# DiltheyLab/MetaMaps

Hardware: AMD Instinct MI355X
Metric: Gbp long reads mapped+classified per sec (whole node), miniSeq+H DB (higher is better)
Workload: dtype u32

## Files before the change

### metamaps_amd/csrc/mm_env.hpp

```cpp
#pragma once
#include <unistd.h>
#include <cstdlib>
#include <cstring>
#include <string>

extern "C" char** environ;

namespace mm {

struct EnvSwitch { const char* name; const char* dflt; const char* kind; const char* what; };

inline const EnvSwitch* env_table(size_t* n) {
  static const EnvSwitch T[] = {
    {"MM_STRICT_ENV", "unset", "user", "refuse MM_* variables that are not in this table (mm_ctx_create returns MM_ERR_ARG, the CLI exits 1)"},
    {"MM_CPU_BUDGET", "min(hardware threads, affinity mask, cgroup CPU quota)", "user", "CPUs the process may keep busy: what every thread pool of the library and the CLI is sized from (cpu_budget.hpp)"},
    {"MM_SYNC", "block when the CPU budget is <= 32, else spin", "user", "how a host thread waits for its stream: \"spin\" (hipStreamSynchronize) or \"block\" (sleep on an event created with hipEventBlockingSync)"},
    {"MM_CLI_WORKERS", "4", "user", "worker contexts per GPU that take read batches in turn (= --workers-per-gpu)"},
    {"MM_CLI_BATCH_READS", "100000", "user", "reads per batch handed to a worker"},
    {"MM_CLI_BATCH_MBASES", "256", "user", "... or this many million bases, whichever comes first"},
    {"MM_CLI_MAP_SLOTS", "2", "tuning", "batches per device that may be inside their mapping section at the same time"},
    {"MM_CLI_BLOCK_BYTES", "128 MiB", "tuning", "block size of the block-parallel FASTQ/FASTA parser over an mmap-ed query file"},
    {"MM_CLI_REF_BLOCK_BYTES", "min(group, 256 MiB)", "tuning", "the same for the reference FASTA"},
    {"MM_CLI_REF_GROUP_BASES", "2^30", "test", "bases per upload group of the reference (small groups: the concat path on small inputs)"},
    {"MM_CLI_REF_SEQUENTIAL", "unset", "test", "reference through the sequential kseq-style reader instead of the block parser"},
    {"MM_BAM_HOST_DECODE", "unset", "test", "BAM query files decoded to ASCII on the host and uploaded like FASTQ (cross-check of the device nt16 packer)"},
    {"MM_CLI_NO_MMAP", "unset", "test", "query and reference files through the sequential reader (what .gz and pipes always take)"},
    {"MM_CLI_NO_PREWARM", "unset", "test", "worker contexts come up with their first batch instead of beside the index build"},
    {"MM_SF_GRID", "the device's CU count", "debug", "resident workgroups of the streaming seed filter (measurement aid: how K3 scales with the CUs at work)"},
    {"MM_CLI_LATE_READER", "unset", "debug", "the query reader starts when the index is built instead of beside the build (measurement aid)"},
    {"MM_CLI_NO_SKETCH_REUSE", "unset", "test", "chunk-major runs recompute minimizers and sketches per chunk (mm_map_batch instead of mm_map_batch_reusing)"},
    {"MM_CLI_NO_HUGE", "unset", "test", "no transparent-huge-page arena for host blocks >= 4 MiB (huge_new.hpp)"},
    {"MM_CLI_FULL_TEARDOWN", "unset", "test", "destroy every object and run static destructors at exit instead of _exit after the last file is closed"},
    {"MM_CLASSIFY_THREADS", "32", "user", "host threads that tokenise the mappings file and format classify's outputs"},
    {"MM_EM_MAX_ITER", "unbounded", "test", "cap on EM iterations in classify (the reference has none)"},
    {"MM_EM_SLICE", "1024", "test", "EM iterations per mm_em_run / mm_em_continue call of classify"},
    {"MM_CLI_TIMING", "unset", "debug", "phase laps of the CLI on stderr (bench.py's e2e legs parse them)"},
    {"MM_CLI_FORMAT_TRACE", "unset", "debug", "per-thread times of the text formatting of a batch on stderr"},
    {"MM_DEVICE_BYTES_CAP", "0 (off)", "test", "the library behaves as if every device had this many bytes: allocations beyond fail, mm_ctx_device_info reports it (placement tests)"},
    {"MM_INDEX_SCALE_MB", "8192", "test", "blocks from this size on are index-scale (pooled per device); a few MB exercise the pool on small inputs"},
    {"MM_NO_SLABS", "unset", "test", "worker buffers are not cut out of pooled index-scale blocks"},
    {"MM_NO_POOL_RESCUE", "unset", "test", "round-3 behaviour: a request the driver refuses hands the whole pool back instead of being served from it"},
    {"MM_RETURN_INDEX_BLOCKS", "unset", "test", "index-scale blocks go back to the driver when released instead of into the device's pool"},
    {"MM_INDEX_PRETRIM", "unset", "test", "a device-filling index build hands the pool back before it starts (round-4 mid-round behaviour)"},
    {"MM_INDEX_NO_PRETRIM", "unset", "test", "... and does not even trim the context's own cache"},
    {"MM_ALLOC_TRACE", "unset", "debug", "every block that comes from the driver, with its cost, on stderr"},
    {"MM_ALLOC_NO_MID_HEADROOM", "unset", "test", "device buffers of 256 KiB .. 64 MiB are asked for without the quarter of headroom that lets later, slightly larger batches reuse them (round 5 behaviour)"},
    {"MM_CTX_TRACE", "unset", "debug", "phases of mm_ctx_create (HIP initialisation, stream, allocator) on stderr"},
    {"MM_HOST_TIMING", "unset", "debug", "host-side sections of mm_map_batch and of the index build on stderr"},
    {"MM_PACK_SCALAR", "unset", "test", "mm_seqset_upload packs bases with the byte-table loop only (cross-check of the AVX2 path, host_pack.cpp)"},
    {"MM_INDEX_PART_MAX", "2^31 - 2^24 entries", "test", "entries per partition of the hash sort (small values: the partitioned sort + merge on small inputs)"},
    {"MM_DUP_SAT", "65535", "test", "saturation value of the stored same-hash neighbour distances (small values: K5's scan fall-back)"},
    {"MM_SKETCH_BITONIC", "unset", "test", "K2 for sketches beyond the LDS radix sort: bitonic network instead of one segmented device sort"},
    {"MM_EAGER_TIEBREAK", "unset", "test", "resolve every duplicate-hash strand by the reference's std::sort order up front instead of only where a strand vote reads one"},
    {"MM_FORCE_AMB_REDO", "unset", "test", "every read with an unresolved strand goes through the redo path"},
    {"MM_NO_HIT_FILTER", "unset", "test", "K3 without the exact seed-hit pre-filter: every hit of every kept list reaches the sort (parity tests of the raw hit list)"},
    {"MM_NO_FUSED_FILTER", "unset", "test", "K3 as probe_kernel + two-pass hit_filter_kernel for every read (what reads that do not fit the fused kernel take)"},
    {"MM_SF_ONESHOT", "unset", "test", "the fused seed filter as one read per workgroup instead of the resident streaming form"},
    {"MM_HF_STAGE_CAP", "auto", "test", "capacity of a read's survivor stage (tiny values: the overflow / re-filter path)"},
    {"MM_HF_WIDE_FROM", "13000", "tuning", "sketch size from which the two-pass filter counts in 32768 position slots instead of 8192"},
    {"MM_HITS_BITONIC", "unset", "test", "K4 hit sort: bitonic / LDS radix per read only, never the segmented device sort"},
    {"MM_SEGSORT_FROM", "auto", "tuning", "hits per read from which K4 uses the segmented device sort"},
    {"MM_L1_SERIAL", "unset", "test", "K4's L1 merge loop as the literal one-thread-per-read loop (cross-check of the wavefront form)"},
    {"MM_L2_FULL", "unset", "test", "K5 evaluates every window (the literal slide) instead of the exact skip-ahead"},
    {"MM_L2_NO_CODES", "unset", "test", "K5 classifies streamed entries again in every pass instead of parking their codes"},
    {"MM_L2_NO_DENSE", "unset", "test", "no dense path for sketches >= 13000 hashes (they take the long-read classes of l2_kernel)"},
    {"MM_L2_DENSE_FROM", "13000", "tuning", "sketch size from which K5 runs as l2_codes_kernel + l2_dense_kernel"},
    {"MM_L2_DENSE_NO_STOP", "unset", "test", "dense path without its early stop (every window evaluated)"},
    {"MM_L2_NO_SMALL_GROUPS", "unset", "test", "groups of fewer than three candidates also run as four-wave workgroups (one launch instead of two)"},
    {"MM_L2_HOST_GROUPS", "unset", "test", "candidate groups formed on the host instead of by l2_group_kernel"},
    {"MM_L2_NO_GROUP_SORT", "unset", "test", "K5 workgroups in read order instead of the order of their candidates' positions"},
    {"MM_L2_GROUP_SORT_MIN", "2048", "tuning", "groups from which the launch order is sorted"},
    {"MM_L2_XCD_ORDER", "unset", "tuning", "deal the position-sorted workgroup list out per XCD (measured: slower, DESIGN.md section 7)"},
    {"MM_L2_V1", "unset", "test", "K5's 10 kb class through l2_kernel (rank codes per entry) instead of the zone kernel l2z_kernel (mm_l2z.hpp): the cross-check and the A/B"},
    {"MM_L2_V1_LONG", "unset", "test", "the long-read classes (sketches of 3 073 .. 13 000 hashes) through l2_kernel, the 10 kb class through the zone kernel"},
    {"MM_L2_SMALL_QLDS", "unset", "tuning", "zone kernel, two-wave workgroups (groups of one or two candidates): the sketch in LDS as in the four-wave workgroups instead of searched in global memory"},
    {"MM_L2_NO_FUSE", "unset", "test", "zone kernel without the band predicted from L1's seed-hit count: its masks always come from a second pass over the stream"},
    {"MM_L2_NO_RANGES", "unset", "test", "the zone kernel's waves search their candidates' index ranges themselves (until round 6) instead of taking them from l2_ranges_kernel (cross-check)"},
    {"MM_L2Z_DBG", "unset", "debug", "zone kernel writes pivot-minus-estimate and its pass count INSTEAD OF RESULTS (tools/l2z_pivot_hist.py; 2: against the predicted estimate)"},
    {"MM_L2_ONE_STREAM", "unset", "test", "the two launches of K5's 10 kb class one behind the other on the context's stream instead of side by side (auxiliary stream)"},
    {"MM_L2_NO_SLOTS", "unset", "test", "K5 scratch indexed by wave number of the launch instead of per-XCD slots taken and given back"},
    {"MM_L2_SLOTS", "auto (resident waves)", "tuning", "number of K5 scratch slots"},
    {"MM_L2_STOP", "0", "debug", "K5 leaves after phase n WITHOUT RESULTS (tools/l2_stop.py)"},
    {"MM_L2_PHASES", "unset", "debug", "K5 phase clocks into its counters (tools/l2_long_phases.py; the zone kernel has them in a build with -DL2Z_CLOCKS only)"},
    {"MM_MZ_DBG", "0", "debug", "K1 leaves after step n WITHOUT RESULTS (tools/stage_ms.py)"},
    {"MM_SF_DBG", "0", "debug", "fused seed filter leaves after phase n WITHOUT RESULTS (tools/sf_dbg.py)"},
    {"MM_HF_DBG", "0", "debug", "two-pass filter leaves after phase n WITHOUT RESULTS"},
    {"MM_SF_PROF", "unset", "debug", "cycle counts per phase of the streaming seed filter on stderr"},
    {"MM_EM_FORCE_COLLECTIVE", "unset", "test", "a one-rank communicator keeps P1-P3' | ncclAllReduce | finalize instead of the plain loop (how one GPU drives the multi-rank path)"},
    {"MM_EM_RESIDENT", "unset", "tuning", "EM as one resident kernel with grid barriers instead of one launch per phase (measured: slower, DESIGN.md section 4)"},
    {"MM_EM_SPLIT", "unset", "test", "with MM_EM_RESIDENT: the phases as launches all the same (cross-check); 2: P2 and P3 in one launch (measured slower than a launch per phase)"},
    {"MM_EM_GRID", "256 (128 resident)", "tuning", "workgroups of the EM kernels"},
    {"MM_EM_BARRIER_TICKS", "2 s", "test", "time-out of the resident kernel's grid barrier before it hands the run to the launch path"},
    {"MM_CLI_FORMAT_PART", "10000", "test", "mapping records per formatter thread of a batch (the text of a batch is formatted in up to eight parts and joined)"},
    {"MM_CLI_CLASSIFY_FROM_FILE", "unset", "test", "mapDirectly --then-classify reads PREFIX back and tokenises it (as `classify` does) instead of taking the lines it has just formatted from memory"},
    {"MM_EM_ORDER", "file", "debug", "\"count\": reads by mapping count for the thread-per-read E step (measurement aid)"},
    {"MM_EM_DBG", "0", "debug", "E-step variants of the round-4 measurements (tools/em_latency.py)"},
    {"MM_EM_PROF", "unset", "debug", "phase clocks of the resident EM kernel on stderr"},
    {"MM_GATHER_SELF_SEND", "unset", "test", "mm_mapping_gather sends the owner's own parts through ncclSend / ncclRecv too (one-GPU test of the exchange)"},
  };
  *n = sizeof T / sizeof T[0];
  return T;
}

inline std::string env_unknown() {
  size_t n = 0; const EnvSwitch* T = env_table(&n);
  std::string bad;
  for (char** e = environ; e && *e; ++e) {
    if (strncmp(*e, "MM_", 3) != 0) continue;
    const char* eq = strchr(*e, '=');
    const std::string name(*e, eq ? (size_t)(eq - *e) : strlen(*e));
    static const char* const outside[] = {"MM_BENCH_", "MM_FUZZ_", "MM_TEST_", "MM_CLI_FUZZ_CASES", "MM_LIB_PATH"};
    bool ours = false;
    for (const char* pfx : outside) ours = ours || name.rfind(pfx, 0) == 0;
    if (ours) continue;
    bool known = false;
    for (size_t i = 0; i < n && !known; ++i) known = name == T[i].name;
    if (!known) bad += (bad.empty() ? "" : ", ") + name;
  }
  return bad;
}
inline bool env_strict() { const char* e = getenv("MM_STRICT_ENV"); return e && *e && strcmp(e, "0") != 0; }

}
```

### metamaps_amd/csrc/mm_l2z.hpp

```cpp
#pragma once
#include "mm_l2.hpp"

namespace mm {

#ifndef L2Z_RING
#define L2Z_RING 128
#endif
__host__ __device__ constexpr int l2z_qcap(bool qlds) { return qlds ? L2Z_RING : 2 * L2Z_RING; }
constexpr int L2Z_QCAP_ = L2Z_RING;
#ifndef L2Z_WAVES_10K
#define L2Z_WAVES_10K 5
#endif
#ifndef L2Z_WAVES_LONG
#define L2Z_WAVES_LONG 4
#endif
__host__ __device__ inline size_t l2z_mask_bytes(int nwq) { return (((size_t)(64 * nwq + 1) * (5 * 8 + 3 * 2)) + 15) & ~(size_t)15; }
__host__ __device__ inline size_t l2z_list_bytes(int nwq) { return (size_t)(64 * 64 * nwq) * 4; }
__host__ __device__ inline int l2z_bloom_log2(int smax) { int b = 15; while (((size_t)1 << b) < (size_t)8 * (size_t)smax && b < 19) ++b; return b; }
__host__ __device__ constexpr int l2z_band(int nwq) { return nwq == 2 ? 128 : 512; }
#ifndef L2Z_CENTRE_SIG
#define L2Z_CENTRE_SIG (-0.70f)
#endif
#ifndef L2Z_CENTRE_SIG_PRED
#define L2Z_CENTRE_SIG_PRED 0.43f
// ... 788 lines not shown
          pm ^= bit;
          if (lane > kk) pm_j ^= bit;
        } else {
          fz += (lane >= zi) ? sign : 0;
          const int at = sign > 0 ? pc - 1 : pc;
          const int fv = __shfl(fz, min(max(at, 0), 63), 64);
          if (sign > 0) { if (pc > 0 && fv >= thr) --pc; }
          else { if (pc < 64 && fv < thr) ++pc; }
          if (lane > kk) pj = pc;
        }
      }
      const bool inw = lane < n_eval;
      const bool outU = inw && pj >= 64;
      const bool outD = inw && has_lo && thr <= z0 - 1;
      const uint64_t um = __ballot(outU), dm = __ballot(outD);
      const bool canU = z0 + 64 < zb + BAND, canD = z0 > zb;
      const uint64_t cut = (canU ? um : 0ull) | (canD ? dm : 0ull);
      const int n_vis = cut ? __builtin_ctzll(cut) : n_eval;
      const uint64_t vis = n_vis >= 64 ? ~0ull : ((1ull << n_vis) - 1ull);
      const uint64_t fu = canU ? 0ull : (um & vis), fd = canD ? 0ull : (dm & vis);
      if ((fu && zdir >= 0) || (fd && zdir <= 0)) {
        const int bk2 = (b + 63 >= blk_end && bk + 1 < nblk) ? bk + 1 : bk;
        if (fu && zdir >= 0) { flag_block(fUpW, bk); flag_block(fUpW, bk2); }
        if (fd && zdir <= 0) { flag_block(fDnW, bk); flag_block(fDnW, bk2); }
      }
      const bool scored = lane < n_vis && !outU && !outD;
      const int sh_j = scored ? sb_j + __popcll(pm_j & ((1ull << (pj & 63)) - 1ull)) : -1;
      const int m = wave_max(sh_j);
      if (m >= 0) {
        const uint64_t at = __ballot(sh_j == m);
        const int j1 = __builtin_ctzll(at), jl = 63 - __builtin_clzll(at);
        auto set_first = [&]() {
          bestR = z0 + __builtin_amdgcn_readlane(pj, j1);
          const int d1 = __builtin_amdgcn_readlane(dj, j1);
          opt_b = b + d1; opt_e = e + __builtin_amdgcn_readlane(aj, j1);
          beg_pos = __builtin_amdgcn_readlane(wpb, d1);
        };
        auto set_last = [&]() {
          const int dl = __builtin_amdgcn_readlane(dj, jl);
          last_b = b + dl; last_pos = __builtin_amdgcn_readlane(wpb, dl);
        };
        if (m > best) { best = m; set_first(); set_last(); }
        else if (m == best && best > 0) {
          if (b + __builtin_amdgcn_readlane(dj, j1) < opt_b) set_first();
          if (b + __builtin_amdgcn_readlane(dj, jl) > last_b) set_last();
        }
        evals += (uint32_t)__popcll(__ballot(scored));
      }
      int dn, an;
      if (n_vis < 64) { dn = __builtin_amdgcn_readlane(dj, n_vis); an = __builtin_amdgcn_readlane(aj, n_vis); }
      else { dn = __builtin_amdgcn_readlane(dj, 63) + __builtin_amdgcn_readlane(hasDel, 63); an = __builtin_amdgcn_readlane(aj, 63) + __builtin_amdgcn_readlane(hasAdd, 63); }
      b += dn; e += an;
      while (b >= blk_end) {
        ++bk;
        if (bk >= nblk || (stage == 1 && bk == j0) || ub_of(bk) < max(best, amin)) { run_stop = true; break; }
        blk_end += bspan;
      }
      if (run_stop) break;
      if (cut) pending_rebuild = true;
      else {
        const int fE = an > 0 ? __builtin_amdgcn_readlane(pE, an - 1) : 0, fB = dn > 0 ? __builtin_amdgcn_readlane(pB, dn - 1) : 0;
        cbase += (fE & 0xffff) - (fB & 0xffff);
        sb += (fE >> 16) - (fB >> 16);
      }
    }
  };

  int zb_first = 0, r_est = 0;
  if (dbg_stop == 9) { release_slot(); return; }
  bool any_pass = ubmax >= amin;
  bool masks_ready = false;
  if (any_pass) {
    const int wo = wo_est;
    const int zb_p = zb, r_ref_p = r_ref;
    r_est = set_band((float)wo, L2Z_CENTRE_SIG);
    if (fused) {
      const int want = zb + BAND / 2;
      masks_ready = zb == zb_p || (want >= zb_p + BAND / 4 && want < zb_p + 3 * BAND / 4);
      if (masks_ready) { zb = zb_p; r_ref = r_ref_p; }
    }
    zb_first = zb;
  }
  while (any_pass) {
    if (++n_pass > (s >> 6) + 4) break;
    if (!masks_ready) { pass_low(); ++n_low; }
    masks_ready = false;
    if (dbg_stop == 6) { release_slot(); return; }
    fill_band_hashes();
    lap(5);
    if (dbg_stop == 7) { release_slot(); return; }
    wave_sync();
    int ub2[2];
    int lane_b = lane;
    asm volatile("" : "+v"(lane_b));
    for (int q = 0; q < 2; ++q) {
      const int bq = lane_b + 64 * q;
      int u = -1;
      const int eLo_q = bq < nblk ? (int)eLoL[bq] : last_end;
      if (bq < nblk && eLo_q < last_end && ((eligW[bq >> 5] >> (bq & 31)) & 1u)) {
        const int bF = bq * bspan, bL = min(bF + bspan - 1, last_end - 1);
        const int eHi_q = (bL + 1 < last_end && bq + 1 < nblk) ? (int)eLoL[bq + 1] : last_end;
        const int a = eLo_q > bL ? pfx(mA, pA, eLo_q) - pfx(mA, pA, bL) : 0;
        u = (r_ref + a >= s) ? pfx(mLo, pLo, eHi_q) - pfx(mLo, pLo, bF) : pfx(mAll, pAll, eHi_q) - pfx(mAll, pAll, bF);
      }
      ub2[q] = u;
    }
    ub2L[lane_b] = (uint16_t)(ub2[0] + 1); ub2L[lane_b + 64] = (uint16_t)(ub2[1] + 1);
    wave_sync();
    int bkmax = 0, done_hi = nblk;
    if (zdir == 0) {
      const int u2max = wave_max(max(ub2[0], ub2[1]));
      const int key2 = max(ub2[0], ub2[1]) == u2max ? ((ub2[0] == u2max) ? lane_b : lane_b + 64) : 1 << 20;
      bkmax = wave_min(key2);
      j0 = bkmax;
      while (j0 > 0 && bkmax - j0 < 3 && 100 * ub_of(j0 - 1) >= 95 * u2max) --j0;
      stage = 0; bk = j0;
    } else { stage = 1; j0 = -1; bk = 0; }
    lap(2);
    if (dbg_stop == 4) { release_slot(); return; }
    for (;;) {
      bool found = false;
      for (;;) {
        if (stage == 1 && bk == j0) bk = done_hi;
        if (bk >= nblk) { if (stage == 0) { done_hi = nblk; stage = 1; bk = 0; continue; } break; }
        if (ub_of(bk) >= max(best, amin)) { found = true; break; }
        if (stage == 0 && bk >= bkmax) { done_hi = bk + 1; stage = 1; bk = 0; continue; }
        ++bk;
      }
      if (!found) break;
      const int nb = bk * bspan;
      blk_end = nb + bspan; run_stop = false;
      b = nb; e = e_of(bk); pending_rebuild = true;
      lap(2);
      block_slide();
      lap(4);
      if (dbg_stop == 8) { release_slot(); return; }
      if (e >= last_end || bk >= nblk) {
        if (stage == 1) break;
        done_hi = nblk; stage = 1; bk = 0;
      }
    }
    wave_sync();
    const bool wantU = __ballot(lane < 4 && fUpW[lane & 3] != 0u) != 0ull, wantD = __ballot(lane < 4 && fDnW[lane & 3] != 0u) != 0ull;
    if (zdir >= 0 && wantU && zb < zb_top) {
      zdir = 1; zb = min(zb + BAND, zb_top);
      r_ref = min(zb + BAND, s) - 1;
      if (lane < 4) { eligW[lane] = fUpW[lane]; fUpW[lane] = 0; }
      continue;
    }
    if (zdir >= 0) { zdir = -1; zb = zb_first; }
    if (wantD && zb > 0) {
      zb = max(0, zb - BAND);
      r_ref = min(zb + BAND, s) - 1;
      if (lane < 4) { eligW[lane] = fDnW[lane]; fDnW[lane] = 0; }
      continue;
    }
    break;
  }

  lap(4);
  if (dbg_stop == 5) { release_slot(); return; }
  int strand = -1, accepted = 0;
  if (best >= amin) {
    accepted = 1;
    int votes = 0, amb_votes = 0;
    const int i0 = pfx(mAll, pAll, opt_b), i1 = pfx(mAll, pAll, opt_e);
    constexpr int VB = 8;
    for (int ib = i0; ib < i1; ib += 64 * VB) {
      uint32_t ew[VB], sq[VB], pwj[VB]; bool cnt_it[VB]; int jv[VB];
#pragma unroll
      for (int u = 0; u < VB; ++u) { const int i = ib + 64 * u + lane; ew[u] = i < i1 ? ML[i] : 0xffffffffu; }
#pragma unroll
      for (int u = 0; u < VB; ++u) {
        const int rk = (int)((ew[u] >> 15) & 0x7fffu);
        jv[u] = (int)(ew[u] & 0x7fffu);
        cnt_it[u] = ew[u] != 0xffffffffu && rk < bestR;
        sq[u] = cnt_it[u] ? (uint32_t)sk_strand[qo + rk] : 0u;
        pwj[u] = cnt_it[u] ? pos[jv[u]].pw : 0u;
      }
#pragma unroll
      for (int u = 0; u < VB; ++u) {
        if (ib + 64 * u >= i1) continue;
        const bool unres = (sq[u] & 2u) && amb_used != nullptr;
        const int contrib = cnt_it[u] ? (((sq[u] & 1u) ? 1 : -1) * pw_strand(pwj[u])) : 0;
        const bool flagged = cnt_it[u] && (pwj[u] & PW_DN);
        int dres = 0;
        if (__ballot(flagged) != 0ull) dres = flagged ? dup_after(I, first0 + jv[u], (int64_t)opt_e - 1 - jv[u]) : 0;
        if (cnt_it[u] && dres == 0) { if (unres) ++amb_votes; else votes += contrib; }
        uint64_t fm = __ballot(dres < 0);
        while (fm) {
          const int l = __builtin_ctzll(fm); fm &= fm - 1;
          const int jj = __builtin_amdgcn_readlane(jv[u], l);
          const uint32_t hj = pos[jj].hash;
          const bool later = wave_has_hash(pos, jj + 1, opt_e, hj, lane);
          if (!later && lane == l) { if (unres) ++amb_votes; else votes += contrib; }
        }
      }
    }
    votes = wave_sum(votes);
    amb_votes = wave_sum(amb_votes);
    if (amb_votes > 0 && ((votes - amb_votes <= 0 && votes + amb_votes > 0) || (dbg_flags & 0x200)) && lane == 0) amb_used[r] = 1;
    strand = votes > 0 ? 1 : -1;
  }
  release_slot();
  if (lane == 0) {
    L2Result o;
    o.contig = contig; o.mean_pos = (beg_pos + last_pos) / 2;
    o.shared = best; o.strand = strand; o.accepted = accepted; o.pad = n_low;
    o.opt_beg = first0 + opt_b; o.opt_end = first0 + opt_e;
    o.n_stream = (uint32_t)M; o.n_evals = evals; o.n_rebuilds = rebuilds; o.pad2 = rounds;
// ... 9 lines not shown
```

### metamaps_amd/csrc/mm_map.hip

```cpp
#include "mm_map.hpp"
#include <functional>
#include <memory>
#include <rocprim/rocprim.hpp>
#include "mm_l2_core.hpp"
#include "mm_l2.hpp"
#include "mm_l2z.hpp"
#include "mm_l2_dense.hpp"
#include <cstdlib>
#include <atomic>
#include <thread>
#include "mm_stats.hpp"
#include <algorithm>
#include <numeric>

namespace mm {

__device__ inline void bitonic_sort_u64(uint64_t* a, int n) {
  for (int k = 2; k <= n; k <<= 1) {
    for (int j = k >> 1; j > 0; j >>= 1) {
      for (int t = threadIdx.x; t < (n >> 1); t += blockDim.x) {
        int i = ((t & ~(j - 1)) << 1) | (t & (j - 1));
        int p = i | j;
        uint64_t x = a[i], y = a[p];
        bool up = (i & k) == 0;
// ... 1645 lines not shown
      };
      if (compact) {
        d_cb.upload(cb.data(), ns, st); d_ce.upload(ce.data(), ns, st);
        DBuf<uint64_t> packed((size_t)run), sorted((size_t)run);
        move_ranges_kernel<<<dim3((unsigned)ns), dim3(256), 0, st>>>(M->hits.p, d_hb.p, d_he.p, packed.p, d_cb.p);
        MM_KERNEL_CHECK();
        seg_sort(packed.p, sorted.p, run, d_cb.p, d_ce.p);
        move_ranges_kernel<<<dim3((unsigned)ns), dim3(256), 0, st>>>(sorted.p, d_cb.p, d_ce.p, M->hits.p, d_hb.p);
        MM_KERNEL_CHECK();
        MM_HIP(mm::stream_sync(st));
      } else {
        DBuf<uint64_t> sorted((size_t)total_hits);
        seg_sort(M->hits.p, sorted.p, (uint64_t)total_hits, d_hb.p, d_he.p);
        move_ranges_kernel<<<dim3((unsigned)ns), dim3(256), 0, st>>>(sorted.p, d_hb.p, d_he.p, M->hits.p, d_hb.p);
        MM_KERNEL_CHECK();
        MM_HIP(mm::stream_sync(st));
      }
    }
    T.end(t_sh);
  }
  hl("K4 launches + sync");
  const size_t t_l1 = T.begin(&M->stats.ms_l1_scan);
  const bool l1_serial = getenv("MM_L1_SERIAL") != nullptr;
  DBuf<uint32_t> cand_n((size_t)n + 1); cand_n.zero(st);
  M->cand_off.alloc((size_t)n + 2);
  const unsigned rblk = (unsigned)ceil_div(std::max<int64_t>(n, 1), 128);
  if (n > 0) {
    if (l1_serial) l1_scan_kernel<false><<<dim3(rblk), dim3(128), 0, st>>>(M->hits.p, M->read_hit_off.p, M->d_read_len.p, M->min_hits.p, n, cand_n.p, nullptr, nullptr, nullptr);
    else l1_wave_kernel<false><<<dim3((unsigned)ceil_div(n, 4)), dim3(256), 0, st>>>(M->hits.p, M->read_hit_off.p, M->d_read_len.p, M->min_hits.p, n, cand_n.p, nullptr, nullptr, nullptr, nullptr);
    MM_KERNEL_CHECK();
  }
  exclusive_scan_u32_u64(cand_n.p, n, M->cand_off.p, scan_tmp, st);
  M->h_cand_off = M->cand_off.to_host(st, (size_t)n + 1);
  hl("L1 count + cand_off download");
  const int64_t ncand = (int64_t)M->h_cand_off[(size_t)n];
  M->n_cand = ncand;
  M->stats.n_candidates = ncand;
  M->cand.alloc((size_t)std::max<int64_t>(3 * ncand, 1));
  M->cand_read.alloc((size_t)std::max<int64_t>(ncand, 1));
  M->l2.alloc((size_t)std::max<int64_t>(ncand, 1));
  DBuf<int32_t> cand_hint((size_t)std::max<int64_t>(ncand, 1));
  DBuf<int64_t> cand_rng;
  const bool no_hint = l1_serial || getenv("MM_L2_NO_FUSE");
  if (no_hint) cand_hint.zero(st);
  M->rec_off.alloc((size_t)n + 1);
  if (ncand > 0) {
    if (l1_serial) l1_scan_kernel<true><<<dim3(rblk), dim3(128), 0, st>>>(M->hits.p, M->read_hit_off.p, M->d_read_len.p, M->min_hits.p, n, nullptr, M->cand_off.p, M->cand.p, M->cand_read.p);
    else l1_wave_kernel<true><<<dim3((unsigned)ceil_div(n, 4)), dim3(256), 0, st>>>(M->hits.p, M->read_hit_off.p, M->d_read_len.p, M->min_hits.p, n, nullptr, M->cand_off.p, M->cand.p, M->cand_read.p, no_hint ? nullptr : cand_hint.p);
    MM_KERNEL_CHECK();
    T.end(t_l1);
    if (!getenv("MM_L2_NO_RANGES")) {
      cand_rng.alloc(2 * (size_t)ncand);
      l2_ranges_kernel<<<dim3((unsigned)ceil_div(ncand, 256)), dim3(256), 0, st>>>(IV, M->cand.p, M->cand_read.p, M->d_read_len.p, ncand, cand_rng.p);
      MM_KERNEL_CHECK();
    }
    MM_REQUIRE(ncand < (1LL << 31), MM_ERR_LIMIT, "more than 2^31 L1 candidates in one batch");
    const int smax = M->smax;
    const char* full_env = getenv("MM_L2_FULL");
    const bool skip = !(full_env && full_env[0] == '1');
    const bool use_dense = !getenv("MM_L2_NO_DENSE");
    const int dense_from = getenv("MM_L2_DENSE_FROM") ? atoi(getenv("MM_L2_DENSE_FROM")) : 13000;
    const bool no_small_groups = getenv("MM_L2_NO_SMALL_GROUPS") != nullptr;
    const bool dev_groups = skip && !getenv("MM_L2_HOST_GROUPS");
    DBuf<int32_t> d_gA0, d_gAn, d_gS0, d_gSn;
    DBuf<unsigned int> grp_ctr(4);
    if (dev_groups) {
      d_gA0.alloc((size_t)ncand); d_gAn.alloc((size_t)ncand); d_gS0.alloc((size_t)ncand); d_gSn.alloc((size_t)ncand);
      grp_ctr.zero(st);
      l2_group_kernel<<<dim3((unsigned)ceil_div(n, 256)), dim3(256), 0, st>>>(M->cand_off.p, M->sk_n.p, M->d_read_len.p, n, P.w + P.k + 1, use_dense ? dense_from : INT_MAX,
                                                                            no_small_groups ? 1 : 0, d_gA0.p, d_gAn.p, d_gS0.p, d_gSn.p, grp_ctr.p);
      MM_KERNEL_CHECK();
    }
    const size_t lds_wide = l2_lds_bytes<uint16_t>(smax, skip, 1, 8);
    std::vector<int32_t> listG; int smG = 0;
    for (int64_t r = 0; r < n && M->stats.n_reads_giant > 0; ++r) {
      const int sr = M->h_sk_n[(size_t)r];
      if (sr < L2_SKETCH_LIMIT) continue;
      smG = std::max(smG, sr);
      for (uint64_t c0 = M->h_cand_off[(size_t)r]; c0 < M->h_cand_off[(size_t)r + 1]; ++c0) listG.push_back((int32_t)c0);
    }
    MM_REQUIRE(lds_wide <= 160 * 1024, MM_ERR_LIMIT, "L2 window state does not fit LDS");
    auto set_lds = [&](const void* fn, size_t bytes) { if (bytes > 64 * 1024) MM_HIP(hipFuncSetAttribute(fn, hipFuncAttributeMaxDynamicSharedMemorySize, (int)bytes)); };
    DBuf<unsigned long long> counters(16); counters.zero(st);
    if (getenv("MM_L2_STOP") || getenv("MM_L2_PHASES") || getenv("MM_FORCE_AMB_REDO") || getenv("MM_L2Z_DBG")) {
      const char* ds = getenv("MM_L2_STOP"); unsigned long long v = (unsigned long long)((ds ? atoi(ds) & 0xff : 0) | (getenv("MM_L2_PHASES") ? 0x100 : 0) | (getenv("MM_FORCE_AMB_REDO") ? 0x200 : 0) | (getenv("MM_L2Z_DBG") ? (atoi(getenv("MM_L2Z_DBG")) == 2 ? 0xc00 : 0x400) : 0)); MM_HIP(hipMemcpyAsync(counters.p + 11, &v, sizeof v, hipMemcpyHostToDevice, st)); MM_HIP(mm::stream_sync(st)); }
    DBuf<int32_t> ovf((size_t)ncand);
    DBuf<unsigned int> ovf_n(1); ovf_n.zero(st);
    DBuf<uint8_t> amb_used;
    if (!lazy_reads.empty()) { amb_used.alloc((size_t)n); amb_used.zero(st); }
    uint8_t* const amb_used_p = lazy_reads.empty() ? nullptr : amb_used.p;
    if (amb_finish) { amb_finish(); amb_finish = nullptr; }
    const size_t t_l2 = T.begin(&M->stats.ms_l2);
    const int force_amb = getenv("MM_FORCE_AMB_REDO") ? 1 : 0;
    auto run_dense = [&](const std::vector<int32_t>& list, int smax_l, uint8_t* amb_ptr) {
      if (list.empty()) return;
      const size_t nl = list.size();
      DBuf<int32_t> d_list(nl); d_list.upload(list.data(), nl, st);
      DBuf<L2Range> d_rng(nl);
      l2_range_kernel<<<dim3((unsigned)ceil_div((int64_t)nl, 4)), dim3(256), 0, st>>>(IV, M->cand.p, M->cand_read.p, M->d_read_len.p, d_list.p, (int)nl, d_rng.p);
      MM_KERNEL_CHECK();
      std::vector<L2Range> rng = d_rng.to_host(st);
      std::vector<uint64_t> coff(nl + 1, 0);
      for (size_t i = 0; i < nl; ++i) coff[i + 1] = coff[i] + (uint64_t)std::max(rng[i].m, 0);
      std::vector<int32_t> cr = M->cand_read.to_host(st, (size_t)ncand);
      std::vector<int32_t> gfirst;
      for (size_t i = 0; i < nl; ++i) if (i == 0 || cr[(size_t)list[i]] != cr[(size_t)list[i - 1]]) gfirst.push_back((int32_t)i);
      gfirst.push_back((int32_t)nl);
      DBuf<uint64_t> d_coff(nl + 1); d_coff.upload(coff.data(), nl + 1, st);
      DBuf<int32_t> d_gf(gfirst.size()); d_gf.upload(gfirst.data(), gfirst.size(), st);
      DBuf<uint32_t> codes((size_t)std::max<uint64_t>(coff[nl], 1));
      const int q_in_lds = smax_l <= LD_Q_LDS_MAX ? 1 : 0;
      const size_t lds = ((size_t)((LD_TSIZE + 3) & ~3) + (q_in_lds ? (size_t)smax_l + 4 : 0)) * 4;
      set_lds((const void*)l2_codes_kernel, lds);
      l2_codes_kernel<<<dim3((unsigned)(gfirst.size() - 1)), dim3(256), lds, st>>>(IV, M->cand_read.p, M->sk_hash.p, M->mz.off.p, M->sk_n.p, d_list.p, d_gf.p,
                                                                                  d_rng.p, d_coff.p, codes.p, q_in_lds);
      MM_KERNEL_CHECK();
      const unsigned slots = (unsigned)std::min<size_t>(nl, (size_t)ctx->cus * 12);
      DBuf<uint32_t> scratch((size_t)slots * l2_dense_slot_words(smax_l));
      DBuf<unsigned int> next(1); next.zero(st);
      l2_dense_kernel<<<dim3(slots), dim3(64), 0, st>>>(IV, M->cand.p, M->cand_read.p, M->sk_strand.p, M->mz.off.p, M->sk_n.p, M->d_read_len.p, M->accept_min.p,
                                                      P.k, P.w, smax_l, M->l2.p, d_list.p, (int)nl, d_rng.p, d_coff.p, codes.p, scratch.p, next.p, amb_ptr, force_amb,
                                                      getenv("MM_L2_DENSE_NO_STOP") ? 0 : 1);
      MM_KERNEL_CHECK();
      MM_HIP(mm::stream_sync(st));
    };
    DBuf<int32_t> d_listG(listG.size());
    DBuf<uint32_t> giant_scratch;
    if (!listG.empty() && use_dense) run_dense(listG, smG, amb_used_p);
    else if (!listG.empty()) {
      d_listG.upload(listG.data(), listG.size(), st);
      const unsigned slots = (unsigned)std::min<size_t>(listG.size(), (size_t)ctx->cus * 8);
      giant_scratch.alloc((size_t)slots * l2_giant_slot_words(smG));
      l2_giant_kernel<<<dim3(slots), dim3(64), 0, st>>>(IV, M->cand.p, M->cand_read.p, M->sk_hash.p, M->sk_strand.p, M->mz.off.p, M->sk_n.p, M->d_read_len.p,
                                                      M->accept_min.p, P.k, P.w, smG, M->l2.p, d_listG.p, (int)listG.size(), giant_scratch.p);
      MM_KERNEL_CHECK();
    }
    if (!skip) {
      std::vector<int32_t> listF;
      for (int64_t r = 0; r < n; ++r) if (M->h_sk_n[(size_t)r] < L2_SKETCH_LIMIT)
        for (uint64_t c0 = M->h_cand_off[(size_t)r]; c0 < M->h_cand_off[(size_t)r + 1]; ++c0) listF.push_back((int32_t)c0);
      DBuf<int32_t> d_listF(listF.size());
      if (!listF.empty()) {
        d_listF.upload(listF.data(), listF.size(), st);
        set_lds((const void*)l2_kernel<false, uint16_t, 1, 8>, lds_wide);
        l2_kernel<false, uint16_t, 1, 8><<<dim3((unsigned)listF.size()), dim3(64), lds_wide, st>>>(IV, M->cand.p, M->cand_read.p, M->sk_hash.p, M->sk_strand.p,
            M->mz.off.p, M->sk_n.p, M->d_read_len.p, M->accept_min.p, P.k, P.w, smax, M->l2.p, counters.p, nullptr, nullptr, d_listF.p, nullptr, nullptr, amb_used_p, nullptr, nullptr, nullptr, 0);
        MM_KERNEL_CHECK();
      }
      MM_HIP(mm::stream_sync(st));
    } else {
      const bool no_slots = getenv("MM_L2_NO_SLOTS") != nullptr;
      const size_t env_slots = getenv("MM_L2_SLOTS") ? ((size_t)std::max(atoi(getenv("MM_L2_SLOTS")), 1) + 7) / 8 * 8 : 0;
      auto max_slots = [&](int nwq) -> size_t { return no_slots ? (size_t)1 << 40 : env_slots ? env_slots : (size_t)ctx->cus * (nwq == 2 ? 64 : 32); };
      DBuf<unsigned int> slot_flags(std::max((size_t)ctx->cus * 64, env_slots)); slot_flags.zero(st);
      unsigned int* const slot_flags_p = no_slots ? nullptr : slot_flags.p;
      auto slots_of = [&](size_t n_waves, int nwq = 8) -> size_t { return std::min((std::max<size_t>(n_waves, 1) + 7) / 8 * 8, max_slots(nwq)); };
      auto masks_for = [&](size_t n_waves, int nwq = 8) -> uint8_t* { return (uint8_t*)ctx->l2_masks_at_least(slots_of(n_waves, nwq) * l2_skip_bytes(nwq)); };
      auto codes_for = [&](size_t n_waves, int nwq) -> void* {
        if (getenv("MM_L2_NO_CODES")) return nullptr;
        return ctx->l2_codes_at_least(slots_of(n_waves, nwq) * (size_t)(64 * 64 * nwq) * (nwq == 2 ? sizeof(uint16_t) : sizeof(uint32_t)));
      };
      const bool v2 = !getenv("MM_L2_V1");
      const bool v2_long = v2 && !getenv("MM_L2_V1_LONG");
      const int32_t* const cand_hint_p = cand_hint.p;
      auto lists_for = [&](size_t n_waves, int nwq) -> void* { return ctx->l2_codes_at_least(slots_of(n_waves, nwq) * l2z_list_bytes(nwq)); };
      auto zmasks_for = [&](size_t n_waves, int nwq) -> uint8_t* { return (uint8_t*)ctx->l2_masks_at_least(slots_of(n_waves, nwq) * l2z_mask_bytes(nwq)); };
      DBuf<int32_t> big((size_t)(v2 ? ncand : 1));
      DBuf<unsigned int> big_n(1); big_n.zero(st);
// ... 80 lines not shown
          if (nS) {
            if (getenv("MM_L2_SMALL_QLDS")) {
              const size_t lds = l2z_lds_bytes(smA, 2, true, bbl, 2);
              set_lds((const void*)l2z_kernel<2, 2, true>, lds);
              l2z_kernel<2, 2, true><<<dim3((unsigned)nS), dim3(128), lds, st_small>>>(IV, M->cand.p, M->cand_read.p, M->sk_hash.p, M->sk_strand.p, M->mz.off.p, M->sk_n.p, M->d_read_len.p,
                  M->accept_min.p, P.k, P.w, smA, bbl, M->l2.p, counters.p, d_gS0.p, d_gSn.p, ovf.p, ovf_n.p, big.p, big_n.p, amb_used_p, (uint32_t*)codes, masks, slot_flags_p, n_slots, cand_hint_p, cand_rng.p);
            } else {
              const size_t lds = l2z_lds_bytes(smA, 2, false, bbl, 2);
              set_lds((const void*)l2z_kernel<2, 2, false>, lds);
              l2z_kernel<2, 2, false><<<dim3((unsigned)nS), dim3(128), lds, st_small>>>(IV, M->cand.p, M->cand_read.p, M->sk_hash.p, M->sk_strand.p, M->mz.off.p, M->sk_n.p, M->d_read_len.p,
                  M->accept_min.p, P.k, P.w, smA, bbl, M->l2.p, counters.p, d_gS0.p, d_gSn.p, ovf.p, ovf_n.p, big.p, big_n.p, amb_used_p, (uint32_t*)codes, masks, slot_flags_p, n_slots, cand_hint_p, cand_rng.p);
            }
            MM_KERNEL_CHECK();
          }
        } else {
        if (nA) {
            const size_t lds = l2_lds_bytes<uint8_t>(smA, true, 4, 2);
            set_lds((const void*)l2_kernel<true, uint8_t, 4, 2>, lds);
            l2_kernel<true, uint8_t, 4, 2><<<dim3((unsigned)nA), dim3(256), lds, st>>>(IV, M->cand.p, M->cand_read.p, M->sk_hash.p, M->sk_strand.p,
                M->mz.off.p, M->sk_n.p, M->d_read_len.p, M->accept_min.p, P.k, P.w, smA, M->l2.p, counters.p, d_gA0.p, d_gAn.p, nullptr, ovf.p, ovf_n.p, amb_used_p, codes, masks, slot_flags_p, n_slots);
            MM_KERNEL_CHECK();
          }
          if (nS) {
            const size_t lds = l2_lds_bytes<uint8_t>(smA, true, 2, 2);
            set_lds((const void*)l2_kernel<true, uint8_t, 2, 2>, lds);
            l2_kernel<true, uint8_t, 2, 2><<<dim3((unsigned)nS), dim3(128), lds, st_small>>>(IV, M->cand.p, M->cand_read.p, M->sk_hash.p, M->sk_strand.p,
                M->mz.off.p, M->sk_n.p, M->d_read_len.p, M->accept_min.p, P.k, P.w, smA, M->l2.p, counters.p, d_gS0.p, d_gSn.p, nullptr, ovf.p, ovf_n.p, amb_used_p, codes, masks, slot_flags_p, n_slots);
            MM_KERNEL_CHECK();
          }
        }
        if (side_by_side) {
          MM_HIP(hipEventRecord(ctx->ev_join, st_small));
          MM_HIP(hipStreamWaitEvent(st, ctx->ev_join, 0));
        }
      }
      if (!gB0.empty()) {
        d_gB0.upload(gB0.data(), gB0.size(), st); d_gBn.upload(gBn.data(), gBn.size(), st);
        sort_by_position(d_gB0, d_gBn, gB0.size());
        if (v2_long) {
          const int bbl = l2z_bloom_log2(smB);
          const size_t lds = l2z_lds_bytes(smB, 8, false, bbl, 4);
          set_lds((const void*)l2z_kernel<4, 8, false>, lds);
          l2z_kernel<4, 8, false><<<dim3((unsigned)gB0.size()), dim3(256), lds, st>>>(IV, M->cand.p, M->cand_read.p, M->sk_hash.p, M->sk_strand.p, M->mz.off.p, M->sk_n.p, M->d_read_len.p,
              M->accept_min.p, P.k, P.w, smB, bbl, M->l2.p, counters.p, d_gB0.p, d_gBn.p, ovf.p, ovf_n.p, big.p, big_n.p, amb_used_p, (uint32_t*)lists_for(gB0.size() * 4, 8), zmasks_for(gB0.size() * 4, 8), slot_flags_p, (int)slots_of(gB0.size() * 4), cand_hint_p, cand_rng.p);
          MM_KERNEL_CHECK();
        } else {
          const size_t lds = l2_lds_bytes<uint8_t>(smB, true, 4, 8);
          set_lds((const void*)l2_kernel<true, uint8_t, 4, 8>, lds);
          l2_kernel<true, uint8_t, 4, 8><<<dim3((unsigned)gB0.size()), dim3(256), lds, st>>>(IV, M->cand.p, M->cand_read.p, M->sk_hash.p, M->sk_strand.p,
              M->mz.off.p, M->sk_n.p, M->d_read_len.p, M->accept_min.p, P.k, P.w, smB, M->l2.p, counters.p, d_gB0.p, d_gBn.p, nullptr, ovf.p, ovf_n.p, amb_used_p, codes_for(gB0.size() * 4, 8), masks_for(gB0.size() * 4), slot_flags_p, (int)slots_of(gB0.size() * 4));
          MM_KERNEL_CHECK();
        }
      }
      DBuf<int32_t> d_gD0(gD0.size()), d_gDn(gDn.size());
      if (!gD0.empty()) {
        d_gD0.upload(gD0.data(), gD0.size(), st); d_gDn.upload(gDn.data(), gDn.size(), st);
        sort_by_position(d_gD0, d_gDn, gD0.size());
        if (v2_long) {
          const int bbl = l2z_bloom_log2(smD);
          const size_t lds = l2z_lds_bytes(smD, 8, false, bbl, 4);
          set_lds((const void*)l2z_kernel<4, 8, false>, lds);
          l2z_kernel<4, 8, false><<<dim3((unsigned)gD0.size()), dim3(256), lds, st>>>(IV, M->cand.p, M->cand_read.p, M->sk_hash.p, M->sk_strand.p, M->mz.off.p, M->sk_n.p, M->d_read_len.p,
              M->accept_min.p, P.k, P.w, smD, bbl, M->l2.p, counters.p, d_gD0.p, d_gDn.p, ovf.p, ovf_n.p, big.p, big_n.p, amb_used_p, (uint32_t*)lists_for(gD0.size() * 4, 8), zmasks_for(gD0.size() * 4, 8), slot_flags_p, (int)slots_of(gD0.size() * 4), cand_hint_p, cand_rng.p);
          MM_KERNEL_CHECK();
        } else {
          const size_t lds = l2_lds_bytes<uint8_t>(smD, true, 4, 8);
          set_lds((const void*)l2_kernel<true, uint8_t, 4, 8>, lds);
          l2_kernel<true, uint8_t, 4, 8><<<dim3((unsigned)gD0.size()), dim3(256), lds, st>>>(IV, M->cand.p, M->cand_read.p, M->sk_hash.p, M->sk_strand.p,
              M->mz.off.p, M->sk_n.p, M->d_read_len.p, M->accept_min.p, P.k, P.w, smD, M->l2.p, counters.p, d_gD0.p, d_gDn.p, nullptr, ovf.p, ovf_n.p, amb_used_p, codes_for(gD0.size() * 4, 8), masks_for(gD0.size() * 4), slot_flags_p, (int)slots_of(gD0.size() * 4));
          MM_KERNEL_CHECK();
        }
      }
      if (!listC.empty()) {
        d_listC.upload(listC.data(), listC.size(), st);
        const size_t lds = l2_lds_bytes<uint16_t>(smC, true, 1, 8);
        set_lds((const void*)l2_kernel<true, uint16_t, 1, 8>, lds);
        l2_kernel<true, uint16_t, 1, 8><<<dim3((unsigned)listC.size()), dim3(64), lds, st>>>(IV, M->cand.p, M->cand_read.p, M->sk_hash.p, M->sk_strand.p,
            M->mz.off.p, M->sk_n.p, M->d_read_len.p, M->accept_min.p, P.k, P.w, smC, M->l2.p, counters.p, nullptr, nullptr, d_listC.p, ovf.p, ovf_n.p, amb_used_p, nullptr, masks_for(listC.size()), slot_flags_p, (int)slots_of(listC.size()));
        MM_KERNEL_CHECK();
      }
      hl("K5 uploads + launches");
      if (M->at_stage) M->at_stage(M->at_stage_user, 2);
      int64_t n_fallback = 0;
      auto run_fallback = [&](uint8_t* amb_ptr) {
        unsigned int h_ovf = 0;
        MM_HIP(hipMemcpyAsync(&h_ovf, ovf_n.p, sizeof h_ovf, hipMemcpyDeviceToHost, st));
        MM_HIP(mm::stream_sync(st));
        if (!h_ovf) return;
        const size_t lds = l2_lds_bytes<uint16_t>(smax, false, 1, 8);
        set_lds((const void*)l2_kernel<false, uint16_t, 1, 8>, lds);
        l2_kernel<false, uint16_t, 1, 8><<<dim3(h_ovf), dim3(64), lds, st>>>(IV, M->cand.p, M->cand_read.p, M->sk_hash.p, M->sk_strand.p,
            M->mz.off.p, M->sk_n.p, M->d_read_len.p, M->accept_min.p, P.k, P.w, smax, M->l2.p, counters.p, nullptr, nullptr, ovf.p, nullptr, nullptr, amb_ptr, nullptr, nullptr, nullptr, 0);
        MM_KERNEL_CHECK();
        ovf_n.zero(st);
        n_fallback += h_ovf;
      };
      int64_t n_big = 0;
      if (v2) {
        unsigned int h_big = 0;
        MM_HIP(hipMemcpyAsync(&h_big, big_n.p, sizeof h_big, hipMemcpyDeviceToHost, st));
        MM_HIP(mm::stream_sync(st));
        if (h_big) {
          const int smW = std::max(std::max(smA, smB), smD);
          const size_t lds = l2_lds_bytes<uint16_t>(smW, true, 1, 8);
          set_lds((const void*)l2_kernel<true, uint16_t, 1, 8>, lds);
          l2_kernel<true, uint16_t, 1, 8><<<dim3(h_big), dim3(64), lds, st>>>(IV, M->cand.p, M->cand_read.p, M->sk_hash.p, M->sk_strand.p,
              M->mz.off.p, M->sk_n.p, M->d_read_len.p, M->accept_min.p, P.k, P.w, smW, M->l2.p, counters.p, nullptr, nullptr, big.p, ovf.p, ovf_n.p, amb_used_p, nullptr, masks_for(h_big), slot_flags_p, (int)slots_of(h_big));
          MM_KERNEL_CHECK();
          n_big = h_big;
        }
      }
      run_fallback(amb_used_p);
      int64_t n_redo = 0;
      if (!lazy_reads.empty()) {
        std::vector<uint8_t> used = amb_used.to_host(st, (size_t)n);
        std::vector<int64_t> fix;
        for (int64_t r : lazy_reads) if (used[(size_t)r]) fix.push_back(r);
        if (!fix.empty()) {
          start_tiebreak(fix)();
          std::vector<int32_t> redo, redoL; int smR = 0, smRL = 0;
          for (int64_t r : fix) {
            const int sr = M->h_sk_n[(size_t)r];
            const bool dense_r = use_dense && (sr >= L2_SKETCH_LIMIT || (sr >= dense_from && M->read_len[(size_t)r] >= P.w + P.k + 1));
            (dense_r ? smRL : smR) = std::max(dense_r ? smRL : smR, sr);
            for (uint64_t c0 = M->h_cand_off[(size_t)r]; c0 < M->h_cand_off[(size_t)r + 1]; ++c0) (dense_r ? redoL : redo).push_back((int32_t)c0);
          }
          run_dense(redoL, smRL, nullptr);
          n_redo += (int64_t)redoL.size();
          DBuf<int32_t> d_redo(std::max<size_t>(redo.size(), 1)); d_redo.upload(redo.data(), redo.size(), st);
          if (!redo.empty()) {
            const size_t lds = l2_lds_bytes<uint16_t>(smR, true, 1, 8);
            set_lds((const void*)l2_kernel<true, uint16_t, 1, 8>, lds);
            l2_kernel<true, uint16_t, 1, 8><<<dim3((unsigned)redo.size()), dim3(64), lds, st>>>(IV, M->cand.p, M->cand_read.p, M->sk_hash.p, M->sk_strand.p,
                M->mz.off.p, M->sk_n.p, M->d_read_len.p, M->accept_min.p, P.k, P.w, smR, M->l2.p, counters.p, nullptr, nullptr, d_redo.p, ovf.p, ovf_n.p, nullptr, nullptr, masks_for(redo.size()), slot_flags_p, (int)slots_of(redo.size()));
            MM_KERNEL_CHECK();
            run_fallback(nullptr);
          }
          MM_HIP(mm::stream_sync(st));
          n_redo += (int64_t)redo.size();
        }
      }
      M->stats.n_l2_wide_redo = n_redo + n_fallback + n_big;
    }
    l2_stats_kernel<<<dim3((unsigned)std::min<int64_t>(ceil_div(ncand, 256), 1024)), dim3(256), 0, st>>>(M->l2.p, ncand, counters.p);
    MM_KERNEL_CHECK();
    T.end(t_l2);
    hl("K5 wait");
    auto hc = counters.to_host(st);
    M->stats.sum_l2_stream_entries = (int64_t)hc[0];
    M->stats.sum_l2_evals = (int64_t)hc[1];
    M->stats.n_l2_rebuilds = (int64_t)hc[2];
    if (getenv("MM_L2_PHASES")) { fprintf(stderr, "l2 rounds %llu zone passes %llu; ", hc[15], hc[12]); fprintf(stderr, "l2 phase clocks [setup passA bounds rebuild slide passB vote]:"); for (int i = 0; i < 7; ++i) fprintf(stderr, " %.3g", (double)hc[3 + i]); fprintf(stderr, "\n"); }
    if (amb_finish) { amb_finish(); amb_finish = nullptr; }
    const size_t t_cp = T.begin(&M->stats.ms_compact);
    DBuf<uint32_t> flag((size_t)ncand);
    DBuf<uint64_t> rank((size_t)ncand + 1);
    accept_flags_kernel<<<dim3((unsigned)ceil_div(ncand, 256)), dim3(256), 0, st>>>(M->l2.p, ncand, flag.p);
    MM_KERNEL_CHECK();
    exclusive_scan_u32_u64(flag.p, ncand, rank.p, scan_tmp, st);
    uint64_t nrec = 0;
    MM_HIP(hipMemcpyAsync(&nrec, rank.p + ncand, sizeof nrec, hipMemcpyDeviceToHost, st));
    MM_HIP(mm::stream_sync(st));
    M->n_rec = (int64_t)nrec;
    M->rec.alloc((size_t)std::max<uint64_t>(nrec, 1));
    write_records_kernel<<<dim3((unsigned)ceil_div(ncand, 256)), dim3(256), 0, st>>>(M->l2.p, M->cand_read.p, M->sk_n.p, flag.p, rank.p, ncand, M->rec.p);
    MM_KERNEL_CHECK();
    read_rec_bounds_kernel<<<dim3((unsigned)ceil_div(n + 1, 256)), dim3(256), 0, st>>>(M->cand_off.p, rank.p, n, M->rec_off.p);
    MM_KERNEL_CHECK();
    T.end(t_cp);
    MM_HIP(mm::stream_sync(st));
  } else {
    T.end(t_l1);
    if (amb_finish) { amb_finish(); amb_finish = nullptr; }
    M->n_rec = 0;
    M->rec.alloc(1);
    M->rec_off.zero(st);
    MM_HIP(mm::stream_sync(st));
  }
  M->h_rec_off = M->rec_off.to_host(st, (size_t)n + 1);
  T.end(t_total);
  T.collect();
  M->stats.n_mappings = M->n_rec;
  for (int64_t r = 0; r < n; ++r) if (M->h_rec_off[(size_t)r + 1] > M->h_rec_off[(size_t)r]) M->stats.n_reads_mapped++;
}

void probed_list_hist(mm_ctx* ctx, const mm_index* I, const mm_mapping* M, int nb, int64_t* hist) {
  hipStream_t st = ctx->stream;
  DBuf<unsigned long long> d((size_t)nb);
  d.zero(st);
  if (M->n_reads > 0)
    probed_list_hist_kernel<<<dim3((unsigned)M->n_reads), dim3(256), 0, st>>>(make_view(I), M->sk_hash.p, M->mz.off.p, M->sk_n.p, nb, d.p);
  MM_KERNEL_CHECK();
  auto h = d.to_host(st);
  for (int i = 0; i < nb; ++i) hist[i] = (int64_t)h[(size_t)i];
}

}
```

Before: 24.04.

## Find next zone block by wave ballots and fold overflow count into one sync

In the 10 kb zone kernel, the serial block-by-block walk that finds the next block whose upper bound passes the threshold is replaced by wave-wide ballots over the per-block bounds, masked for the already-swept range. The pass-count guard now hands the candidate back to l2_kernel via the big list instead of just breaking out. On the host, the overflow counter is read in the same copy and sync as the big-list count, which saves one round trip. Two env switches are added for cross-checks, and the ballot masks add some risk of off-by-one errors at block boundaries.

```diff
diff --git a/metamaps_amd/csrc/mm_env.hpp b/metamaps_amd/csrc/mm_env.hpp
--- a/metamaps_amd/csrc/mm_env.hpp
+++ b/metamaps_amd/csrc/mm_env.hpp
@@ -76,6 +76,8 @@
     {"MM_L2_SMALL_QLDS", "unset", "tuning", "zone kernel, two-wave workgroups (groups of one or two candidates): the sketch in LDS as in the four-wave workgroups instead of searched in global memory"},
     {"MM_L2_NO_FUSE", "unset", "test", "zone kernel without the band predicted from L1's seed-hit count: its masks always come from a second pass over the stream"},
     {"MM_L2_NO_RANGES", "unset", "test", "the zone kernel's waves search their candidates' index ranges themselves (until round 6) instead of taking them from l2_ranges_kernel (cross-check)"},
+    {"MM_L2Z_FORCE_HANDBACK", "unset", "test", "the zone kernel hands every candidate that reaches its band loop to l2_kernel, as its pass-count guard does (the hand-back path against the default)"},
+    {"MM_L2Z_WALK_SEARCH", "unset", "test", "the 10 kb zone kernel finds the next block to sweep by the walk one block at a time (the long-read classes' way) instead of by ballots: the same blocks, the cross-check"},
     {"MM_L2Z_DBG", "unset", "debug", "zone kernel writes pivot-minus-estimate and its pass count INSTEAD OF RESULTS (tools/l2z_pivot_hist.py; 2: against the predicted estimate)"},
     {"MM_L2_ONE_STREAM", "unset", "test", "the two launches of K5's 10 kb class one behind the other on the context's stream instead of side by side (auxiliary stream)"},
     {"MM_L2_NO_SLOTS", "unset", "test", "K5 scratch indexed by wave number of the launch instead of per-XCD slots taken and given back"},
diff --git a/metamaps_amd/csrc/mm_l2z.hpp b/metamaps_amd/csrc/mm_l2z.hpp
--- a/metamaps_amd/csrc/mm_l2z.hpp
+++ b/metamaps_amd/csrc/mm_l2z.hpp
@@ -894,7 +894,11 @@
     zb_first = zb;
   }
   while (any_pass) {
-    if (++n_pass > (s >> 6) + 4) break;
+    if (++n_pass > (s >> 6) + 4 || (dbg_flags & 0x1000)) {
+      release_slot();
+      if (lane == 0) { L2Result z{}; out[c] = z; big_list[atomicAdd(big_n, 1u)] = (int32_t)c; }
+      return;
+    }
     if (!masks_ready) { pass_low(); ++n_low; }
     masks_ready = false;
     if (dbg_stop == 6) { release_slot(); return; }
@@ -930,14 +934,43 @@
     } else { stage = 1; j0 = -1; bk = 0; }
     lap(2);
     if (dbg_stop == 4) { release_slot(); return; }
+    auto passing_from = [&](int from, int thr, uint64_t& p0, uint64_t& p1) {
+      const int u0 = (int)ub2L[lane_b] - 1, u1 = (int)ub2L[lane_b + 64] - 1;
+      p0 = __ballot(u0 >= thr && lane_b >= from);
+      p1 = __ballot(u1 >= thr && lane_b + 64 >= from);
+    };
+    auto first_of = [&](uint64_t p0, uint64_t p1) -> int { return p0 ? __builtin_ctzll(p0) : (p1 ? 64 + __builtin_ctzll(p1) : 1 << 20); };
     for (;;) {
       bool found = false;
-      for (;;) {
-        if (stage == 1 && bk == j0) bk = done_hi;
-        if (bk >= nblk) { if (stage == 0) { done_hi = nblk; stage = 1; bk = 0; continue; } break; }
-        if (ub_of(bk) >= max(best, amin)) { found = true; break; }
-        if (stage == 0 && bk >= bkmax) { done_hi = bk + 1; stage = 1; bk = 0; continue; }
-        ++bk;
+      if (NWQ == 2 && !(dbg_flags & 0x2000)) {
+        const int thr = max(best, amin);
+        uint64_t p0, p1;
+        if (stage == 0) {
+          passing_from(bk, thr, p0, p1);
+          const int f = first_of(p0, p1), g = max(bk, bkmax);
+          if (g < f && g < nblk) { done_hi = g + 1; stage = 1; bk = 0; }
+          else if (f < nblk) { bk = f; found = true; }
+          else { done_hi = nblk; stage = 1; bk = 0; }
+        }
+        if (stage == 1 && !found) {
+          passing_from(bk, thr, p0, p1);
+          if (bk <= j0) {
+            const uint64_t k0 = (j0 > 0 ? (j0 >= 64 ? ~0ull : (1ull << j0) - 1ull) : 0ull) | (done_hi >= 64 ? 0ull : ~0ull << done_hi);
+            const int j1 = j0 - 64, d1 = done_hi - 64;
+            const uint64_t k1 = (j1 > 0 ? (j1 >= 64 ? ~0ull : (1ull << j1) - 1ull) : 0ull) | (d1 <= 0 ? ~0ull : (d1 >= 64 ? 0ull : ~0ull << d1));
+            p0 &= k0; p1 &= k1;
+          }
+          const int f = first_of(p0, p1);
+          if (f < nblk) { bk = f; found = true; }
+        }
+      } else {
+        for (;;) {
+          if (stage == 1 && bk == j0) bk = done_hi;
+          if (bk >= nblk) { if (stage == 0) { done_hi = nblk; stage = 1; bk = 0; continue; } break; }
+          if (ub_of(bk) >= max(best, amin)) { found = true; break; }
+          if (stage == 0 && bk >= bkmax) { done_hi = bk + 1; stage = 1; bk = 0; continue; }
+          ++bk;
+        }
       }
       if (!found) break;
       const int nb = bk * bspan;
diff --git a/metamaps_amd/csrc/mm_map.hip b/metamaps_amd/csrc/mm_map.hip
--- a/metamaps_amd/csrc/mm_map.hip
+++ b/metamaps_amd/csrc/mm_map.hip
@@ -1751,8 +1751,8 @@
     MM_REQUIRE(lds_wide <= 160 * 1024, MM_ERR_LIMIT, "L2 window state does not fit LDS");
     auto set_lds = [&](const void* fn, size_t bytes) { if (bytes > 64 * 1024) MM_HIP(hipFuncSetAttribute(fn, hipFuncAttributeMaxDynamicSharedMemorySize, (int)bytes)); };
     DBuf<unsigned long long> counters(16); counters.zero(st);
-    if (getenv("MM_L2_STOP") || getenv("MM_L2_PHASES") || getenv("MM_FORCE_AMB_REDO") || getenv("MM_L2Z_DBG")) {
-      const char* ds = getenv("MM_L2_STOP"); unsigned long long v = (unsigned long long)((ds ? atoi(ds) & 0xff : 0) | (getenv("MM_L2_PHASES") ? 0x100 : 0) | (getenv("MM_FORCE_AMB_REDO") ? 0x200 : 0) | (getenv("MM_L2Z_DBG") ? (atoi(getenv("MM_L2Z_DBG")) == 2 ? 0xc00 : 0x400) : 0)); MM_HIP(hipMemcpyAsync(counters.p + 11, &v, sizeof v, hipMemcpyHostToDevice, st)); MM_HIP(mm::stream_sync(st)); }
+    if (getenv("MM_L2_STOP") || getenv("MM_L2_PHASES") || getenv("MM_FORCE_AMB_REDO") || getenv("MM_L2Z_DBG") || getenv("MM_L2Z_FORCE_HANDBACK") || getenv("MM_L2Z_WALK_SEARCH")) {
+      const char* ds = getenv("MM_L2_STOP"); unsigned long long v = (unsigned long long)((ds ? atoi(ds) & 0xff : 0) | (getenv("MM_L2_PHASES") ? 0x100 : 0) | (getenv("MM_FORCE_AMB_REDO") ? 0x200 : 0) | (getenv("MM_L2Z_DBG") ? (atoi(getenv("MM_L2Z_DBG")) == 2 ? 0xc00 : 0x400) : 0) | (getenv("MM_L2Z_FORCE_HANDBACK") ? 0x1000 : 0) | (getenv("MM_L2Z_WALK_SEARCH") ? 0x2000 : 0)); MM_HIP(hipMemcpyAsync(counters.p + 11, &v, sizeof v, hipMemcpyHostToDevice, st)); MM_HIP(mm::stream_sync(st)); }
     DBuf<int32_t> ovf((size_t)ncand);
     DBuf<unsigned int> ovf_n(1); ovf_n.zero(st);
     DBuf<uint8_t> amb_used;
@@ -1999,10 +1999,11 @@
       hl("K5 uploads + launches");
       if (M->at_stage) M->at_stage(M->at_stage_user, 2);
       int64_t n_fallback = 0;
-      auto run_fallback = [&](uint8_t* amb_ptr) {
-        unsigned int h_ovf = 0;
-        MM_HIP(hipMemcpyAsync(&h_ovf, ovf_n.p, sizeof h_ovf, hipMemcpyDeviceToHost, st));
-        MM_HIP(mm::stream_sync(st));
+      auto run_fallback = [&](uint8_t* amb_ptr, bool read_ovf, unsigned int h_ovf) {
+        if (read_ovf) {
+          MM_HIP(hipMemcpyAsync(&h_ovf, ovf_n.p, sizeof h_ovf, hipMemcpyDeviceToHost, st));
+          MM_HIP(mm::stream_sync(st));
+        }
         if (!h_ovf) return;
         const size_t lds = l2_lds_bytes<uint16_t>(smax, false, 1, 8);
         set_lds((const void*)l2_kernel<false, uint16_t, 1, 8>, lds);
@@ -2013,9 +2014,11 @@
         n_fallback += h_ovf;
       };
       int64_t n_big = 0;
+      unsigned int h_ovf0 = 0;
       if (v2) {
         unsigned int h_big = 0;
         MM_HIP(hipMemcpyAsync(&h_big, big_n.p, sizeof h_big, hipMemcpyDeviceToHost, st));
+        MM_HIP(hipMemcpyAsync(&h_ovf0, ovf_n.p, sizeof h_ovf0, hipMemcpyDeviceToHost, st));
         MM_HIP(mm::stream_sync(st));
         if (h_big) {
           const int smW = std::max(std::max(smA, smB), smD);
@@ -2027,7 +2030,7 @@
           n_big = h_big;
         }
       }
-      run_fallback(amb_used_p);
+      run_fallback(amb_used_p, !v2, h_ovf0);
       int64_t n_redo = 0;
       if (!lazy_reads.empty()) {
         std::vector<uint8_t> used = amb_used.to_host(st, (size_t)n);
@@ -2051,7 +2054,7 @@
             l2_kernel<true, uint16_t, 1, 8><<<dim3((unsigned)redo.size()), dim3(64), lds, st>>>(IV, M->cand.p, M->cand_read.p, M->sk_hash.p, M->sk_strand.p,
                 M->mz.off.p, M->sk_n.p, M->d_read_len.p, M->accept_min.p, P.k, P.w, smR, M->l2.p, counters.p, nullptr, nullptr, d_redo.p, ovf.p, ovf_n.p, nullptr, nullptr, masks_for(redo.size()), slot_flags_p, (int)slots_of(redo.size()));
             MM_KERNEL_CHECK();
-            run_fallback(nullptr);
+            run_fallback(nullptr, true, 0);
           }
           MM_HIP(mm::stream_sync(st));
           n_redo += (int64_t)redo.size();
```

After: 25.39, median of 6. 1.06x the previous value.
